# MMintLab/gelslim_depth

Measured on AMD Instinct MI355X. Metric: train frames/sec (320x427) at batch 32, higher is better.
Workload: dtype f32

## Files before the change

### gelslim_depth_amd/csrc/gsd_wgrad_w2d.hip

```cpp
#include "gsd_common.h"
#include "gsd_wgrad_internal.h"
#include <type_traits>

#include <cstdio>
#include <cstdlib>

typedef float f32x2d __attribute__((ext_vector_type(2)));

struct WgW2dParams {
  SrcD a0, a1;
  SrcD dy;
  float* slabs;
  int M, Ncols;
  int N, H, W;
  int KY, KX, kx_log2;
  int tiles_y, tiles_x, sy_n, sx_n;
  int WR, NP, NI;
  int ksteps_total, splits, mblocks, nblocks;
};

__device__ __forceinline__ float w2d_dpp(float v, const int ctrl_is_pair) {
  return ctrl_is_pair ? __builtin_bit_cast(float, __builtin_amdgcn_update_dpp(0, __builtin_bit_cast(int, v), 0xB1, 0xf, 0xf, true))
                      : __builtin_bit_cast(float, __builtin_amdgcn_update_dpp(0, __builtin_bit_cast(int, v), 0x5A, 0xf, 0xf, true));
}

template <int NWM, int NWN, bool PLAIN>
__global__ __launch_bounds__(512, 1) void wgrad3x3_w2d_kernel(const WgW2dParams P) {
  static_assert(NWM * NWN == 8, "8-wave blocks");
  constexpr int BM = 32 * NWM, BN = 16 * NWN;
  constexpr bool UROW = BM == 64;
  constexpr int NV = BN / 32;
  constexpr int TSU = BM * 24 + 4, TSV = BN * 24 + 4;
  constexpr int BUF = 4 * TSU + 4 * TSV;
  constexpr int NPD = UROW ? 1 : 2;
  constexpr int WINI = BN == 32 ? 10 : 20;
  constexpr int KB = BN == 32 ? 2 : 3;
  constexpr int WIN = NPD * 8 * 256;
  constexpr int IMG = WIN + 2 * WINI * 256;
  extern __shared__ __attribute__((aligned(16))) float smem[];

  const int tid = threadIdx.x, lane = tid & 63;
  const int wave = __builtin_amdgcn_readfirstlane(tid >> 6);
  const int wm = wave / NWN, wn = wave % NWN;
  const int j = lane >> 4, l16 = lane & 15;

  const int lid = xcd_swizzle(blockIdx.x, gridDim.x);
  const int per_split = P.mblocks * P.nblocks;
  const int split = lid / per_split;
  const int rem = lid - split * per_split;
  const int mb = rem % P.mblocks, nb = rem / P.mblocks;
  const int m0 = mb * BM, n0 = nb * BN;
  const int s_begin = (int)((long long)split * P.ksteps_total / P.splits);
  const int s_end = (int)((long long)(split + 1) * P.ksteps_total / P.splits);
  const int nst = s_end - s_begin;

  const bool seg1 = P.a1.C > 0 && n0 >= P.a0.C;
  const float* const S_p = seg1 ? P.a1.p : P.a0.p;
  const long long S_ns = seg1 ? P.a1.ns : P.a0.ns, S_cs = seg1 ? P.a1.cs : P.a0.cs;
  const int S_H = seg1 ? P.a1.H : P.a0.H, S_W = seg1 ? P.a1.W : P.a0.W, S_ws = seg1 ? P.a1.ws : P.a0.ws;
  const int S_oh = seg1 ? P.a1.oh : P.a0.oh, S_ow = seg1 ? P.a1.ow : P.a0.ow;
  const int S_c0 = n0 - (seg1 ? P.a0.C : 0);

  const int kxm = P.KX - 1;
  const int u_t = UROW ? (tid >> 1) & 3 : tid & 3;
  const int u_r = UROW ? tid & 1 : 0;
  const int u_co = UROW ? tid >> 3 : tid >> 2;
  const int u_tyl = u_t >> P.kx_log2, u_txl = u_t & kxm;
  const unsigned u_voff = (unsigned)((long long)u_co * P.dy.cs + (long long)(2 * u_tyl + u_r) * P.dy.ws + 4 * u_txl) * 4u;
  const unsigned u_wr = (unsigned)(IMG + u_t * TSU + u_co * 24) * 4u;
  const int v_kr = tid & 3, v_t = (tid >> 2) & 3, v_ci = tid >> 4;
  const int v_tyl = v_t >> P.kx_log2, v_txl = v_t & kxm;
  const unsigned v_rd = (unsigned)(WIN + ((v_ci * P.WR + 2 * v_tyl + v_kr) * P.NP + v_txl) * 4) * 4u;
  const unsigned v_wr = (unsigned)(IMG + 4 * TSU + v_t * TSV + v_ci * 24 + v_kr * 6) * 4u;
  int geo_packed = u_tyl | u_txl << 3 | v_tyl << 6 | v_txl << 9 | v_kr << 12 | u_r << 15;
  asm volatile("" : "+v"(geo_packed));
  const float v_sgn = (tid & 3) == 1 ? 1.f : -1.f;
  const float u_sgn = (UROW && (tid & 1)) ? -1.f : 1.f;
  constexpr int SCS = IMG + 2 * BUF;
  float lo = -__builtin_inff();
  if constexpr (!PLAIN) {
    const SrcD& S = seg1 ? P.a1 : P.a0;
    if (tid < BN) {
      f32x2d v = f32x2d{1.f, 0.f};
      if (S.scale != nullptr) v = f32x2d{S.scale[S_c0 + tid], S.shift[S_c0 + tid]};
      *reinterpret_cast<f32x2d*>(smem + SCS + 2 * tid) = v;
    }
    if (S.relu) lo = 0.f;
  }

  int st_n, st_sy, st_sx;
  {
    const int per = P.sy_n * P.sx_n;
    st_n = s_begin / per;
    const int rs = s_begin - st_n * per;
    st_sy = rs / P.sx_n;
    st_sx = rs - st_sy * P.sx_n;
  }

  int r_mask = 0;
  bool r_edge = false;
  float* const raw_w = smem + wave * 256;
  const float* const raw_r = smem + wave * 256 + lane * 4;
  unsigned x_off[KB];
  int x_meta = 0;
  {
    const int per_ch = P.WR * P.NP;
#pragma unroll
    for (int k = 0; k < KB; ++k) {
      const int pid = 64 * (wave + 8 * k) + lane;
      const int ch = pid / per_ch, rem = pid - ch * per_ch;
      const int wr = rem / P.NP, pp = rem - wr * P.NP;
      const bool dummy = ch >= BN;
      x_off[k] = dummy ? 0u : (unsigned)((long long)ch * S_cs + (long long)wr * S_ws + 4 * pp) * 4u;
      x_meta |= (dummy ? 128 : (wr | pp << 4)) << (8 * k);
    }
    asm volatile("" : "+v"(x_meta));
  }

  auto load = [&](auto wb_c) __attribute__((always_inline)) {
    constexpr int wb = decltype(wb_c)::value;
    const int n = st_n, ty0 = st_sy * P.KY, tx0 = st_sx * P.KX;
    if (++st_sx == P.sx_n) {
      st_sx = 0;
      if (++st_sy == P.sy_n) {
        st_sy = 0;
        ++st_n;
      }
    }
    const char* const dblk = reinterpret_cast<const char*>(P.dy.p + (long long)n * P.dy.ns + (long long)m0 * P.dy.cs);
    const char* vblk = reinterpret_cast<const char*>(S_p + (long long)n * S_ns + (long long)S_c0 * S_cs) - 16;
    asm volatile("" : "+s"(vblk));
    const int hs = 2 * ty0 - 1 - S_oh, wsx = 4 * tx0 - 1 - S_ow;
    const unsigned d_org = (unsigned)(2 * ty0 * P.dy.ws + 4 * tx0) * 4u;
    const int v_org = (hs * S_ws + wsx) * 4 + 16;
    const bool tiles_in = ty0 + P.KY <= P.tiles_y && tx0 + P.KX <= P.tiles_x;
    const bool inside = tiles_in && 2 * (ty0 + P.KY) <= P.H && hs >= 0 && hs + 2 * P.KY + 2 <= S_H && wsx >= 0 &&
                        wsx + 4 * P.KX + 2 <= S_W;
    r_edge = !inside;
    unsigned o_y0 = d_org + u_voff, o_y1 = o_y0 + (unsigned)P.dy.ws * 4u;
    if (!inside) {
      int m = 0;
      int geo = geo_packed;
      asm volatile("" : "+v"(geo));
      {
        const int ty = ty0 + (geo & 7), tx = tx0 + (geo >> 3 & 7);
        const bool t_ok = ty < P.tiles_y && tx < P.tiles_x;
        const int h = 2 * ty + (geo >> 15 & 1);
        const bool ok0 = t_ok && h < P.H, ok1 = t_ok && h + 1 < P.H;
        o_y0 = ok0 ? o_y0 : 0u;
        o_y1 = ok1 ? o_y1 : 0u;
        m = (ok0 ? 1 : 0) | (ok1 ? 2 : 0);
      }
      {
        const int vy = geo >> 6 & 7, vx = geo >> 9 & 7;
        const int ty = ty0 + vy, tx = tx0 + vx;
        const bool t_ok = ty < P.tiles_y && tx < P.tiles_x;
        const int row = hs + 2 * vy + (geo >> 12 & 3), c0 = wsx + 4 * vx;
        const bool r_ok = t_ok && (unsigned)row < (unsigned)S_H;
        const int lo_ = c0 < 0 ? -c0 : 0, hi_ = S_W - c0;
        const int lo = lo_ < 6 ? lo_ : 6, hi = hi_ < 0 ? 0 : (hi_ < 6 ? hi_ : 6);
        const int cm = (r_ok && hi > lo) ? ((1 << hi) - 1) & ~((1 << lo) - 1) : 0;
        m |= cm << 2;
      }
      r_mask = m;
    }
    auto fill = [&](const char* base, unsigned off, float* dst) __attribute__((always_inline)) {
      __builtin_amdgcn_global_load_lds(reinterpret_cast<const float*>(base + off), dst, 16, 0, 0);
    };
#pragma unroll
    for (int k = 0; k < KB; ++k)
      if (wave + 8 * k < P.NI) {
        unsigned off = (unsigned)v_org + x_off[k];
        if (!inside) {
          int mt = x_meta;
          asm volatile("" : "+v"(mt));
          mt >>= 8 * k;
          const int row = hs + (mt & 15), c0 = wsx + 4 * (mt >> 4 & 7);
          const bool ok = !(mt & 128) && (unsigned)row < (unsigned)S_H && c0 + 3 >= 0 && c0 < S_W;
          off = ok ? off : 0u;
        }
        fill(vblk, off, smem + WIN + wb * (WINI * 256) + (wave + 8 * k) * 256);
      }
    __builtin_amdgcn_s_waitcnt(0xC07F);
    fill(dblk, o_y0, raw_w);
    if constexpr (!UROW) fill(dblk, o_y1, raw_w + 8 * 256);
  };

  auto transform = [&](auto buf_c) __attribute__((always_inline)) {
    constexpr int buf = decltype(buf_c)::value;
    const f32x2d p1m1 = {1.f, -1.f}, p2m2 = {2.f, -2.f}, c4 = {4.f, 4.f};
    auto a4_row = [&](const f32x4& y, f32x2d& u12, f32x2d& u34) __attribute__((always_inline)) {
      const f32x2d lo2 = {y[0], y[1]}, hi2 = {y[2], y[3]};
      const f32x2d pq = lo2 + hi2;
      const f32x2d ab = __builtin_elementwise_fma(c4, hi2, lo2);
      u12 = __builtin_elementwise_fma(f32x2d{pq[1], pq[1]}, p1m1, f32x2d{pq[0], pq[0]});
      u34 = __builtin_elementwise_fma(f32x2d{ab[1], ab[1]}, p2m2, f32x2d{ab[0], ab[0]});
    };
    {
      f32x4 y0 = *reinterpret_cast<const f32x4*>(raw_r), y1 = y0;
      if constexpr (!UROW) y1 = *reinterpret_cast<const f32x4*>(raw_r + 8 * 256);
      if (r_edge) {
        if (!(r_mask & 1)) y0 = f32x4{0.f, 0.f, 0.f, 0.f};
        if constexpr (!UROW)
          if (!(r_mask & 2)) y1 = f32x4{0.f, 0.f, 0.f, 0.f};
      }
      f32x2d a12, a34;
      a4_row(y0, a12, a34);
      if constexpr (UROW) {
        const f32x2d sg = {u_sgn, u_sgn};
        const f32x2d a05 = {y0[0], y0[3]};
        const f32x2d x12 = {w2d_dpp(a12[0], 1), w2d_dpp(a12[1], 1)}, x34 = {w2d_dpp(a34[0], 1), w2d_dpp(a34[1], 1)};
        const f32x2d x05 = {w2d_dpp(a05[0], 1), w2d_dpp(a05[1], 1)};
        const f32x2d t12 = __builtin_elementwise_fma(a12, sg, x12), t34 = __builtin_elementwise_fma(a34, sg, x34);
        const f32x2d t05 = __builtin_elementwise_fma(a05, sg, x05);
        float* const o_own = reinterpret_cast<float*>(reinterpret_cast<char*>(smem) + u_wr) + buf * BUF + ((tid & 1) ? 18 : 0);
        float* const o_t1 = reinterpret_cast<float*>(reinterpret_cast<char*>(smem) + u_wr) + buf * BUF + ((tid & 1) ? 12 : 6);
        *reinterpret_cast<f32x2d*>(o_own) = a12;
        *reinterpret_cast<f32x2d*>(o_own + 2) = a34;
        *reinterpret_cast<f32x2d*>(o_own + 4) = a05;
        *reinterpret_cast<f32x2d*>(o_t1) = t12;
        *reinterpret_cast<f32x2d*>(o_t1 + 2) = t34;
        *reinterpret_cast<f32x2d*>(o_t1 + 4) = t05;
      } else {
        f32x2d b12, b34;
        a4_row(y1, b12, b34);
        const f32x2d s12 = a12 + b12, s34 = a34 + b34, d12 = a12 - b12, d34 = a34 - b34;
        const float s0 = y0[0] + y1[0], s5 = y0[3] + y1[3], d0 = y0[0] - y1[0], d5 = y0[3] - y1[3];
        float* const op = reinterpret_cast<float*>(reinterpret_cast<char*>(smem) + u_wr) + buf * BUF;
        *reinterpret_cast<f32x4*>(op) = f32x4{a12[0], a12[1], a34[0], a34[1]};
        *reinterpret_cast<f32x4*>(op + 4) = f32x4{y0[0], y0[3], s12[0], s12[1]};
        *reinterpret_cast<f32x4*>(op + 8) = f32x4{s34[0], s34[1], s0, s5};
        *reinterpret_cast<f32x4*>(op + 12) = f32x4{d12[0], d12[1], d34[0], d34[1]};
        *reinterpret_cast<f32x4*>(op + 16) = f32x4{d0, d5, b12[0], b12[1]};
        *reinterpret_cast<f32x4*>(op + 20) = f32x4{b34[0], b34[1], y1[0], y1[3]};
      }
    }
#pragma unroll
    for (int i = 0; i < NV; ++i) {
      const float* const wp = reinterpret_cast<const float*>(reinterpret_cast<const char*>(smem) + v_rd) + buf * (WINI * 256) + i * 32 * (P.WR * P.NP * 4);
      const f32x4 ra = *reinterpret_cast<const f32x4*>(wp);
      const f32x2d rb = *reinterpret_cast<const f32x2d*>(wp + 4);
      f32x2d t0 = {ra[0], ra[1]}, t1 = {ra[2], ra[3]}, t2 = rb;
      if constexpr (!PLAIN) {
        const f32x2d ss = *reinterpret_cast<const f32x2d*>(smem + SCS + 2 * ((tid >> 4) + 32 * i));
        const f32x2d sc2 = {ss[0], ss[0]}, sh2 = {ss[1], ss[1]}, lo2 = {lo, lo};
        t0 = __builtin_elementwise_max(__builtin_elementwise_fma(t0, sc2, sh2), lo2);
        t1 = __builtin_elementwise_max(__builtin_elementwise_fma(t1, sc2, sh2), lo2);
        t2 = __builtin_elementwise_max(__builtin_elementwise_fma(t2, sc2, sh2), lo2);
      }
      if (r_edge) {
        const int m = r_mask;
        if (!(m & 4)) t0[0] = 0.f;
        if (!(m & 8)) t0[1] = 0.f;
        if (!(m & 16)) t1[0] = 0.f;
        if (!(m & 32)) t1[1] = 0.f;
        if (!(m & 64)) t2[0] = 0.f;
        if (!(m & 128)) t2[1] = 0.f;
      }
      const f32x2d m41 = {-4.f, -1.f}, m5 = {-5.f, -5.f};
      const f32x2d ac = __builtin_elementwise_fma(f32x2d{t1[0], t1[0]}, m41, f32x2d{t2[0], t2[0]});
      const f32x2d be = __builtin_elementwise_fma(f32x2d{t0[1], t0[1]}, m41, f32x2d{t1[1], t1[1]});
      const f32x2d v12 = __builtin_elementwise_fma(f32x2d{be[0], be[0]}, p1m1, f32x2d{ac[0], ac[0]});
      const f32x2d v34 = __builtin_elementwise_fma(f32x2d{be[1], be[1]}, p2m2, f32x2d{ac[1], ac[1]});
      const f32x2d v05 = __builtin_elementwise_fma(t0, c4, __builtin_elementwise_fma(t1, m5, t2));
      const f32x2d sg = {v_sgn, v_sgn};
      const f32x2d x12 = {w2d_dpp(v12[0], 0), w2d_dpp(v12[1], 0)}, x34 = {w2d_dpp(v34[0], 0), w2d_dpp(v34[1], 0)};
      const f32x2d x05 = {w2d_dpp(v05[0], 0), w2d_dpp(v05[1], 0)};
      float* const op = reinterpret_cast<float*>(reinterpret_cast<char*>(smem) + v_wr) + buf * BUF + i * (32 * 24);
      *reinterpret_cast<f32x2d*>(op) = __builtin_elementwise_fma(sg, x12, v12);
      *reinterpret_cast<f32x2d*>(op + 2) = __builtin_elementwise_fma(sg, x34, v34);
      *reinterpret_cast<f32x2d*>(op + 4) = __builtin_elementwise_fma(sg, x05, v05);
    }
  };

  f32x4 acc[2][24];

  const int a_rd = IMG + j * TSU + (wm * 32 + l16) * 24;
  const int b_rd = IMG + 4 * TSU + j * TSV + (wn * 16 + l16) * 24;

  using I0 = std::integral_constant<int, 0>;
  using I1 = std::integral_constant<int, 1>;
  if (nst > 0) {
    load(I0{});
    gsd_dma_barrier();
    transform(I0{});
    if (nst > 1) load(I1{});
    gsd_dma_barrier();
  }
#pragma unroll
  for (int m = 0; m < 2; ++m)
#pragma unroll
    for (int f = 0; f < 24; ++f) acc[m][f] = f32x4{0.f, 0.f, 0.f, 0.f};
  if (nst > 0) {
    auto step = [&](const int it, auto cur_c) __attribute__((always_inline)) {
      constexpr int cur = decltype(cur_c)::value, nxt = cur ^ 1;
      const bool tr = it + 1 < nst, ld = it + 2 < nst;
      const float* const Sb = smem + cur * BUF;
      const f32x2d p1m1 = {1.f, -1.f}, p2m2 = {2.f, -2.f}, c4 = {4.f, 4.f};
      f32x4 a0, a1, b;
      auto rd_ops = [&](const int g) __attribute__((always_inline)) {
        a0 = *reinterpret_cast<const f32x4*>(Sb + a_rd + 4 * g);
        a1 = *reinterpret_cast<const f32x4*>(Sb + a_rd + 16 * 24 + 4 * g);
        b = *reinterpret_cast<const f32x4*>(Sb + b_rd + 4 * g);
      };
      auto mm = [&](const int g) __attribute__((always_inline)) {
#pragma unroll
        for (int e = 0; e < 4; ++e) {
          acc[0][4 * g + e] = mfma16(a0[e], b[e], acc[0][4 * g + e]);
          acc[1][4 * g + e] = mfma16(a1[e], b[e], acc[1][4 * g + e]);
        }
      };
      auto a4_row = [&](const f32x4& y, f32x2d& u12, f32x2d& u34) __attribute__((always_inline)) {
        const f32x2d lo2 = {y[0], y[1]}, hi2 = {y[2], y[3]};
        const f32x2d pq = lo2 + hi2;
        const f32x2d ab = __builtin_elementwise_fma(c4, hi2, lo2);
        u12 = __builtin_elementwise_fma(f32x2d{pq[1], pq[1]}, p1m1, f32x2d{pq[0], pq[0]});
        u34 = __builtin_elementwise_fma(f32x2d{ab[1], ab[1]}, p2m2, f32x2d{ab[0], ab[0]});
      };
      const int t_mask = r_mask;
      const bool t_edge = r_edge;
      f32x4 y0, y1;
      f32x2d a12, a34, b12, b34;
      f32x4 ra;
      f32x2d rb, v12, v34, v05;
      float* const u_out = reinterpret_cast<float*>(reinterpret_cast<char*>(smem) + u_wr) + nxt * BUF;
      auto rd_y = [&]() __attribute__((always_inline)) {
        y0 = *reinterpret_cast<const f32x4*>(raw_r);
        y1 = y0;
        if constexpr (!UROW) y1 = *reinterpret_cast<const f32x4*>(raw_r + 8 * 256);
      };
      auto u_rows = [&]() __attribute__((always_inline)) {
        if (t_edge) {
          if (!(t_mask & 1)) y0 = f32x4{0.f, 0.f, 0.f, 0.f};
          if constexpr (!UROW)
            if (!(t_mask & 2)) y1 = f32x4{0.f, 0.f, 0.f, 0.f};
        }
        a4_row(y0, a12, a34);
        if constexpr (!UROW) a4_row(y1, b12, b34);
      };
      auto u_cols = [&]() __attribute__((always_inline)) {
        if constexpr (UROW) {
          const f32x2d sg = {u_sgn, u_sgn};
          const f32x2d a05 = {y0[0], y0[3]};
          const f32x2d x12 = {w2d_dpp(a12[0], 1), w2d_dpp(a12[1], 1)}, x34 = {w2d_dpp(a34[0], 1), w2d_dpp(a34[1], 1)};
          const f32x2d x05 = {w2d_dpp(a05[0], 1), w2d_dpp(a05[1], 1)};
          float* const o_own = u_out + ((tid & 1) ? 18 : 0);
          float* const o_t1 = u_out + ((tid & 1) ? 12 : 6);
          *reinterpret_cast<f32x2d*>(o_own) = a12;
          *reinterpret_cast<f32x2d*>(o_own + 2) = a34;
          *reinterpret_cast<f32x2d*>(o_own + 4) = a05;
          *reinterpret_cast<f32x2d*>(o_t1) = __builtin_elementwise_fma(a12, sg, x12);
          *reinterpret_cast<f32x2d*>(o_t1 + 2) = __builtin_elementwise_fma(a34, sg, x34);
          *reinterpret_cast<f32x2d*>(o_t1 + 4) = __builtin_elementwise_fma(a05, sg, x05);
        } else {
          const f32x2d s12 = a12 + b12, s34 = a34 + b34, d12 = a12 - b12, d34 = a34 - b34;
          const float s0 = y0[0] + y1[0], s5 = y0[3] + y1[3], d0 = y0[0] - y1[0], d5 = y0[3] - y1[3];
          *reinterpret_cast<f32x4*>(u_out) = f32x4{a12[0], a12[1], a34[0], a34[1]};
          *reinterpret_cast<f32x4*>(u_out + 4) = f32x4{y0[0], y0[3], s12[0], s12[1]};
          *reinterpret_cast<f32x4*>(u_out + 8) = f32x4{s34[0], s34[1], s0, s5};
          *reinterpret_cast<f32x4*>(u_out + 12) = f32x4{d12[0], d12[1], d34[0], d34[1]};
          *reinterpret_cast<f32x4*>(u_out + 16) = f32x4{d0, d5, b12[0], b12[1]};
          *reinterpret_cast<f32x4*>(u_out + 20) = f32x4{b34[0], b34[1], y1[0], y1[3]};
        }
      };
      auto rd_v = [&](const int i) __attribute__((always_inline)) {
        const float* const wp = reinterpret_cast<const float*>(reinterpret_cast<const char*>(smem) + v_rd) + nxt * (WINI * 256) + i * 32 * (P.WR * P.NP * 4);
        ra = *reinterpret_cast<const f32x4*>(wp);
        rb = *reinterpret_cast<const f32x2d*>(wp + 4);
      };
      auto v_rows = [&](const int i) __attribute__((always_inline)) {
        f32x2d t0 = {ra[0], ra[1]}, t1 = {ra[2], ra[3]}, t2 = rb;
        if constexpr (!PLAIN) {
          const f32x2d ss = *reinterpret_cast<const f32x2d*>(smem + SCS + 2 * ((tid >> 4) + 32 * i));
          const f32x2d sc2 = {ss[0], ss[0]}, sh2 = {ss[1], ss[1]}, lo2 = {lo, lo};
          t0 = __builtin_elementwise_max(__builtin_elementwise_fma(t0, sc2, sh2), lo2);
          t1 = __builtin_elementwise_max(__builtin_elementwise_fma(t1, sc2, sh2), lo2);
          t2 = __builtin_elementwise_max(__builtin_elementwise_fma(t2, sc2, sh2), lo2);
        }
        if (t_edge) {
          const int m = t_mask;
          if (!(m & 4)) t0[0] = 0.f;
          if (!(m & 8)) t0[1] = 0.f;
          if (!(m & 16)) t1[0] = 0.f;
          if (!(m & 32)) t1[1] = 0.f;
          if (!(m & 64)) t2[0] = 0.f;
          if (!(m & 128)) t2[1] = 0.f;
        }
        const f32x2d m41 = {-4.f, -1.f}, m5 = {-5.f, -5.f};
        const f32x2d ac = __builtin_elementwise_fma(f32x2d{t1[0], t1[0]}, m41, f32x2d{t2[0], t2[0]});
        const f32x2d be = __builtin_elementwise_fma(f32x2d{t0[1], t0[1]}, m41, f32x2d{t1[1], t1[1]});
        v12 = __builtin_elementwise_fma(f32x2d{be[0], be[0]}, p1m1, f32x2d{ac[0], ac[0]});
        v34 = __builtin_elementwise_fma(f32x2d{be[1], be[1]}, p2m2, f32x2d{ac[1], ac[1]});
        v05 = __builtin_elementwise_fma(t0, c4, __builtin_elementwise_fma(t1, m5, t2));
      };
      auto v_cols = [&](const int i) __attribute__((always_inline)) {
        int tq = threadIdx.x;
        asm volatile("" : "+v"(tq));
        const float sgn = (tq & 3) == 1 ? 1.f : -1.f;
        const f32x2d sg = {sgn, sgn};
        const f32x2d x12 = {w2d_dpp(v12[0], 0), w2d_dpp(v12[1], 0)}, x34 = {w2d_dpp(v34[0], 0), w2d_dpp(v34[1], 0)};
        const f32x2d x05 = {w2d_dpp(v05[0], 0), w2d_dpp(v05[1], 0)};
        float* const op = reinterpret_cast<float*>(reinterpret_cast<char*>(smem) + v_wr) + nxt * BUF + i * (32 * 24);
        *reinterpret_cast<f32x2d*>(op) = __builtin_elementwise_fma(sg, x12, v12);
        *reinterpret_cast<f32x2d*>(op + 2) = __builtin_elementwise_fma(sg, x34, v34);
        *reinterpret_cast<f32x2d*>(op + 4) = __builtin_elementwise_fma(sg, x05, v05);
      };
      auto group = [&](const int g, auto piece) __attribute__((always_inline)) {
        mm(g);
        __builtin_amdgcn_sched_barrier(0);
        if (g + 1 < 6) rd_ops(g + 1);
        piece();
        __builtin_amdgcn_sched_barrier(0);
      };
      rd_ops(0);
      if (tr) rd_y();
      __builtin_amdgcn_sched_barrier(0);
      group(0, [&]() __attribute__((always_inline)) { if (ld) load(cur_c); });
      group(1, [&]() __attribute__((always_inline)) { if (tr) { u_rows(); if constexpr (UROW) u_cols(); } });
      group(2, [&]() __attribute__((always_inline)) { if (tr) { rd_v(0); if constexpr (!UROW) u_cols(); } });
      group(3, [&]() __attribute__((always_inline)) { if (tr) v_rows(0); });
      group(4, [&]() __attribute__((always_inline)) { if (tr) { v_cols(0); if constexpr (NV > 1) rd_v(1); } });
      group(5, [&]() __attribute__((always_inline)) {
        if constexpr (NV > 1) {
          if (tr) { v_rows(1); v_cols(1); }
        }
      });
      gsd_dma_barrier();
    };
    for (int it = 0; it < nst; it += 2) {
      step(it, I0{});
      if (it + 1 < nst) step(it + 1, I1{});
    }
  }

  const size_t pl = (size_t)P.M * P.Ncols;
  int tid_e = threadIdx.x;
  asm volatile("" : "+v"(tid_e));
  const int j_e = (tid_e & 63) >> 4, l16_e = tid_e & 15;
#pragma unroll
  for (int m = 0; m < 2; ++m)
#pragma unroll
    for (int reg = 0; reg < 4; ++reg) {
      const int mr = m0 + wm * 32 + m * 16 + j_e * 4 + reg;
      const int col = n0 + wn * 16 + l16_e;
      float E[4][3];
#pragma unroll
      for (int fr = 0; fr < 4; ++fr) {
        const float D1 = acc[m][fr * 6 + 0][reg], D2 = acc[m][fr * 6 + 1][reg], D3 = acc[m][fr * 6 + 2][reg];
        const float D4 = acc[m][fr * 6 + 3][reg], D0 = acc[m][fr * 6 + 4][reg], D5 = acc[m][fr * 6 + 5][reg];
        E[fr][0] = 0.25f * D0 - (1.f / 6.f) * (D1 + D2) + (1.f / 24.f) * (D3 + D4);
        E[fr][1] = (1.f / 6.f) * (D2 - D1) + (1.f / 12.f) * (D3 - D4);
        E[fr][2] = (1.f / 6.f) * (D3 + D4 - D1 - D2) + D5;
      }
      float* const o = P.slabs + ((size_t)split * 9 * P.M + mr) * P.Ncols + col;
#pragma unroll
      for (int s = 0; s < 3; ++s) {
        const float h = 0.5f * (E[1][s] + E[2][s]);
        o[(0 * 3 + s) * pl] = E[0][s] + h;
        o[(1 * 3 + s) * pl] = 0.5f * (E[1][s] - E[2][s]);
        o[(2 * 3 + s) * pl] = h + E[3][s];
      }
    }
}

namespace {

struct WgW2dPlan {
  int KY, KX, kx_log2, tiles_y, tiles_x, sy_n, sx_n, BM, BN, mblocks, nblocks, ksteps_total, splits;
  int64_t slab_elems;
  bool ok;
};

WgW2dPlan plan_wg2d(int N, int H, int W, int M, int Ncols) {
  WgW2dPlan p;
  p.tiles_y = ceil_div(H, 2);
  p.tiles_x = ceil_div(W, 4);
  long best = -1;
  const int force_kx = gsd_env_int("GSD_WG2D_KX", 0);
  for (int kx = 4; kx >= 1; kx /= 2) {
    if (force_kx && kx != force_kx) continue;
    const int ky = 4 / kx;
    const long steps = (long)ceil_div(p.tiles_y, ky) * ceil_div(p.tiles_x, kx) * (kx == 4 ? 100 : kx == 2 ? 99 : 112);
    if (best < 0 || steps < best) {
      best = steps;
      p.KY = ky; p.KX = kx;
    }
  }
  p.kx_log2 = p.KX == 4 ? 2 : p.KX == 2 ? 1 : 0;
  p.sy_n = ceil_div(p.tiles_y, p.KY);
  p.sx_n = ceil_div(p.tiles_x, p.KX);
  p.BM = M >= 128 ? 128 : 64;
  p.BN = p.BM == 128 ? 32 : 64;
  p.ok = M % p.BM == 0 && Ncols % p.BN == 0;
  p.mblocks = ceil_div(M, p.BM);
  p.nblocks = ceil_div(Ncols, p.BN);
  p.ksteps_total = N * p.sy_n * p.sx_n;
  const int target = gsd_env_int("GSD_WG2D_BLOCKS", 256);
  int splits = ceil_div(target, p.mblocks * p.nblocks);
  if (splits > p.ksteps_total) splits = p.ksteps_total;
  if (splits > 2048) splits = 2048;
  if (splits < 1) splits = 1;
  p.splits = splits;
  p.slab_elems = (int64_t)splits * 9 * M * Ncols;
  return p;
}

}

int64_t gsd_wgrad_w2d_workspace(int N, int H, int W, int Cin, int Cout) {
  const WgW2dPlan p = plan_wg2d(N, H, W, Cout, Cin);
  return p.ok ? p.slab_elems : 0;
}

int64_t gsd_wgrad_w2d_mfma_count(int N, int H, int W, int Cin, int Cout) {
  const WgW2dPlan p = plan_wg2d(N, H, W, Cout, Cin);
  return p.ok ? (int64_t)p.ksteps_total * 24 * (Cout / 16) * (Cin / 16) : 0;
}

int gsd_wgrad_w2d_use(const gsd_src* a, int nsrc, const gsd_src* dy, int Cin, int Cout, int N, int H, int W) {
  if (gsd_env_int("GSD_WGRAD_W2D", 1) == 0) return 0;
  const WgW2dPlan p = plan_wg2d(N, H, W, Cout, Cin);
  if (!p.ok) return 0;
  if (dy->w_stride % 4 != 0 || ((uintptr_t)dy->ptr & 15) != 0 || dy->c_stride % 4 != 0 || dy->n_stride % 4 != 0) return 0;
  if (dy->w_stride < 4 * p.tiles_x) return 0;
  if ((int64_t)p.BM * dy->c_stride * 4 >= (1LL << 31)) return 0;
  if (nsrc == 2 && a[0].C % p.BN != 0) return 0;
  for (int i = 0; i < nsrc; ++i) {
    if (a[i].slack < 4) return 0;
    if ((int64_t)p.BN * a[i].c_stride * 4 >= (1LL << 31)) return 0;
    if ((int64_t)(a[i].H + 4) * a[i].w_stride * 4 >= (1LL << 31)) return 0;
  }
  return 1;
}

int gsd_wgrad_w2d_run(const gsd_src* a, int nsrc, const gsd_src* dy, int Cin, int Cout, float* workspace, int64_t workspace_elems,
                      int N, int H, int W, int* splits_out, void* stream) {
  const WgW2dPlan pl = plan_wg2d(N, H, W, Cout, Cin);
  GSD_REQUIRE(pl.ok, GSD_ERR_UNSUPPORTED, "gsd_conv3x3_wgrad (w2d): shape not served");
  GSD_REQUIRE(workspace_elems >= pl.slab_elems, GSD_ERR_WORKSPACE, "gsd_conv3x3_wgrad: workspace %lld < %lld elements",
              (long long)workspace_elems, (long long)pl.slab_elems);
  WgW2dParams P;
  P.a0 = to_srcd(a[0]);
  P.a1 = nsrc > 1 ? to_srcd(a[1]) : null_srcd();
  P.dy = to_srcd(*dy);
  P.slabs = workspace;
  P.M = Cout; P.Ncols = Cin;
  P.N = N; P.H = H; P.W = W;
  P.KY = pl.KY; P.KX = pl.KX; P.kx_log2 = pl.kx_log2;
  P.tiles_y = pl.tiles_y; P.tiles_x = pl.tiles_x; P.sy_n = pl.sy_n; P.sx_n = pl.sx_n;
  P.WR = 2 * pl.KY + 2; P.NP = pl.KX + 1;
  P.NI = (pl.BN * P.WR * P.NP + 63) / 64;
  P.ksteps_total = pl.ksteps_total; P.splits = pl.splits; P.mblocks = pl.mblocks; P.nblocks = pl.nblocks;
  bool plain = true;
  for (int i = 0; i < nsrc; ++i) plain = plain && a[i].scale == nullptr && a[i].relu == 0;
  const long grid = (long)pl.splits * pl.mblocks * pl.nblocks;
  const size_t lds = ((size_t)(pl.BM == 64 ? 1 : 2) * 8 * 256 + (size_t)2 * (pl.BN == 32 ? 10 : 20) * 256 +
                      (size_t)2 * (4 * (pl.BM * 24 + 4) + 4 * (pl.BN * 24 + 4)) + 2 * pl.BN) * sizeof(float);
  GSD_REQUIRE(P.NI <= 8 * (pl.BN == 32 ? 2 : 3) && P.NI <= (pl.BN == 32 ? 10 : 20), GSD_ERR_UNSUPPORTED, "gsd_conv3x3_wgrad (w2d): window image too large");
  if (gsd_env_set("GSD_WG43_TRACE"))
    fprintf(stderr, "wg2d M%d N%d %dx%d B%d kstep %dx%d ksteps %d splits %d blocks %ld BM %d BN %d plain %d lds %zu\n", Cout, Cin, H, W,
            N, pl.KY, pl.KX, pl.ksteps_total, pl.splits, grid, pl.BM, pl.BN, (int)plain, lds);
  const dim3 g((int)grid);
  const hipStream_t st = (hipStream_t)stream;
  const char* const what = "gsd_conv3x3_wgrad (w2d)";
  if (int e = pl.BM == 128 ? (plain ? gsd_launch<wgrad3x3_w2d_kernel<4, 2, true>>(what, g, dim3(512), lds, st, P)
                                    : gsd_launch<wgrad3x3_w2d_kernel<4, 2, false>>(what, g, dim3(512), lds, st, P))
                           : (plain ? gsd_launch<wgrad3x3_w2d_kernel<2, 4, true>>(what, g, dim3(512), lds, st, P)
                                    : gsd_launch<wgrad3x3_w2d_kernel<2, 4, false>>(what, g, dim3(512), lds, st, P)))
    return e;
  *splits_out = pl.splits;
  return GSD_OK;
}
```

Measured before the change: 382.5.

## Precompute edge masks, branchless load masking, and restructure LDS transform stores in Winograd wgrad

Replaces per-step boundary checks in the Winograd 3x3 weight-gradient kernel with per-thread row/column mask tables computed once. Each k-step is classified as first, last or second-to-last, and zeroing is done with bitwise masks instead of branches. The U/V transform stores are reorganised into a new LDS record layout addressed through raw LDS pointers, and the epilogue is remapped to match. The step loop drops its per-iteration tr/ld guards, and the default block target becomes the CU count. The code adds stricter eligibility checks on source offsets and NI, and carries a correctness risk if the remapped layout or mask tables miss a boundary case.

```diff
diff --git a/gelslim_depth_amd/csrc/gsd_wgrad_w2d.hip b/gelslim_depth_amd/csrc/gsd_wgrad_w2d.hip
--- a/gelslim_depth_amd/csrc/gsd_wgrad_w2d.hip
+++ b/gelslim_depth_amd/csrc/gsd_wgrad_w2d.hip
@@ -6,6 +6,11 @@
 #include <cstdlib>
 
 typedef float f32x2d __attribute__((ext_vector_type(2)));
+
+template <class T>
+__device__ __forceinline__ __attribute__((address_space(3))) T* wg_lds(unsigned byte_addr) {
+  return (__attribute__((address_space(3))) T*)(size_t)byte_addr;
+}
 
 struct WgW2dParams {
   SrcD a0, a1;
@@ -18,6 +23,20 @@
   int WR, NP, NI;
   int ksteps_total, splits, mblocks, nblocks;
 };
+
+__device__ __forceinline__ int wg_bit_mask(int m, const int bit) {
+  int k = (m << (31 - bit)) >> 31;
+  asm volatile("" : "+v"(k));
+  return k;
+}
+__device__ __forceinline__ float wg_keep(float x, int m, const int bit) {
+  return __builtin_bit_cast(float, __builtin_bit_cast(int, x) & wg_bit_mask(m, bit));
+}
+__device__ __forceinline__ f32x4 wg_keep4(const f32x4 x, int m, const int bit) {
+  typedef int i32x4w __attribute__((ext_vector_type(4)));
+  const int k = wg_bit_mask(m, bit);
+  return __builtin_bit_cast(f32x4, __builtin_bit_cast(i32x4w, x) & i32x4w{k, k, k, k});
+}
 
 __device__ __forceinline__ float w2d_dpp(float v, const int ctrl_is_pair) {
   return ctrl_is_pair ? __builtin_bit_cast(float, __builtin_amdgcn_update_dpp(0, __builtin_bit_cast(int, v), 0xB1, 0xf, 0xf, true))
@@ -66,16 +85,20 @@
   const int u_r = UROW ? tid & 1 : 0;
   const int u_co = UROW ? tid >> 3 : tid >> 2;
   const int u_tyl = u_t >> P.kx_log2, u_txl = u_t & kxm;
-  const unsigned u_voff = (unsigned)((long long)u_co * P.dy.cs + (long long)(2 * u_tyl + u_r) * P.dy.ws + 4 * u_txl) * 4u;
-  const unsigned u_wr = (unsigned)(IMG + u_t * TSU + u_co * 24) * 4u;
+  unsigned u_voff = (unsigned)((long long)u_co * P.dy.cs + (long long)(2 * u_tyl + u_r) * P.dy.ws + 4 * u_txl) * 4u;
+  const unsigned smem_b = (unsigned)(size_t)(__attribute__((address_space(3))) void*)smem;
+  const unsigned u_rec = smem_b + (unsigned)(IMG + u_t * TSU + u_co * 24) * 4u;
+  const unsigned u_wr = u_rec + (UROW ? 16u * u_r : 0u);
+  const unsigned u_ws = u_rec + 64u + 4u * u_r;
   const int v_kr = tid & 3, v_t = (tid >> 2) & 3, v_ci = tid >> 4;
   const int v_tyl = v_t >> P.kx_log2, v_txl = v_t & kxm;
-  const unsigned v_rd = (unsigned)(WIN + ((v_ci * P.WR + 2 * v_tyl + v_kr) * P.NP + v_txl) * 4) * 4u;
-  const unsigned v_wr = (unsigned)(IMG + 4 * TSU + v_t * TSV + v_ci * 24 + v_kr * 6) * 4u;
-  int geo_packed = u_tyl | u_txl << 3 | v_tyl << 6 | v_txl << 9 | v_kr << 12 | u_r << 15;
-  asm volatile("" : "+v"(geo_packed));
-  const float v_sgn = (tid & 3) == 1 ? 1.f : -1.f;
-  const float u_sgn = (UROW && (tid & 1)) ? -1.f : 1.f;
+  const unsigned v_rd = smem_b + (unsigned)(WIN + ((v_ci * P.WR + 2 * v_tyl + v_kr) * P.NP + v_txl) * 4) * 4u;
+  const int v_slot = (0x1320 >> (4 * v_kr)) & 3;
+  const unsigned v_rec = smem_b + (unsigned)(IMG + 4 * TSU + v_t * TSV + v_ci * 24) * 4u;
+  const unsigned v_wr = v_rec + 16u * v_slot;
+  const unsigned v_ws = v_rec + 64u + 16u * (v_slot >> 1) + 4u * (v_slot & 1);
+  float v_sgn = (tid & 3) == 1 ? 1.f : -1.f;
+  float u_sgn = (UROW && (tid & 1)) ? -1.f : 1.f;
   constexpr int SCS = IMG + 2 * BUF;
   float lo = -__builtin_inff();
   if constexpr (!PLAIN) {
@@ -98,12 +121,17 @@
   }
 
   int r_mask = 0;
-  bool r_edge = false;
+  int r_edge = 0;
+  int st_left = nst - 1;
   float* const raw_w = smem + wave * 256;
   const float* const raw_r = smem + wave * 256 + lane * 4;
   unsigned x_off[KB];
-  int x_meta = 0;
+  auto fill_bit = [](const int k) { return k < 2 ? 256 << k : 2; };
+  int row_tab, col_tab;
+  const int sy_l2 = P.sy_n > 2 && 2 * (P.sy_n - 1) * P.KY + 1 - S_oh > S_H ? P.sy_n - 2 : -1;
+  const int sx_l2 = P.sx_n > 2 && 4 * (P.sx_n - 1) * P.KX + 1 - S_ow > S_W ? P.sx_n - 2 : -1;
   {
+    int x_wr[KB], x_pp[KB];
     const int per_ch = P.WR * P.NP;
 #pragma unroll
     for (int k = 0; k < KB; ++k) {
@@ -112,20 +140,57 @@
       const int wr = rem / P.NP, pp = rem - wr * P.NP;
       const bool dummy = ch >= BN;
       x_off[k] = dummy ? 0u : (unsigned)((long long)ch * S_cs + (long long)wr * S_ws + 4 * pp) * 4u;
-      x_meta |= (dummy ? 128 : (wr | pp << 4)) << (8 * k);
-    }
-    asm volatile("" : "+v"(x_meta));
+      x_wr[k] = dummy ? -1 : wr;
+      x_pp[k] = pp;
+    }
+    auto row_field = [&](const int ty0) {
+      const int hs = 2 * ty0 - 1 - S_oh;
+      const int uty = ty0 + u_tyl, h = 2 * uty + u_r;
+      int f = (uty < P.tiles_y && h < P.H ? 1 : 0) | (!UROW && uty < P.tiles_y && h + 1 < P.H ? 2 : 0);
+      if (ty0 + v_tyl < P.tiles_y && (unsigned)(hs + 2 * v_tyl + v_kr) < (unsigned)S_H) f |= 0xFC;
+#pragma unroll
+      for (int k = 0; k < KB; ++k)
+        if (x_wr[k] >= 0 && (unsigned)(hs + x_wr[k]) < (unsigned)S_H) f |= fill_bit(k);
+      return f;
+    };
+    auto col_field = [&](const int tx0) {
+      const int wsx = 4 * tx0 - 1 - S_ow;
+      int f = tx0 + u_txl < P.tiles_x ? (UROW ? 1 : 3) : 0;
+      const int c0 = wsx + 4 * v_txl;
+      const int lo_ = c0 < 0 ? -c0 : 0, hi_ = S_W - c0;
+      const int lo = lo_ < 6 ? lo_ : 6, hi = hi_ < 0 ? 0 : (hi_ < 6 ? hi_ : 6);
+      if (tx0 + v_txl < P.tiles_x && hi > lo) f |= (((1 << hi) - 1) & ~((1 << lo) - 1)) << 2;
+#pragma unroll
+      for (int k = 0; k < KB; ++k) {
+        const int ck = wsx + 4 * x_pp[k];
+        if (x_wr[k] >= 0 && ck + 3 >= 0 && ck < S_W) f |= fill_bit(k);
+      }
+      return f;
+    };
+    row_tab = row_field(0) | row_field((P.sy_n - 1) * P.KY) << 10 | row_field((P.sy_n > 2 ? P.sy_n - 2 : 0) * P.KY) << 20;
+    col_tab = col_field(0) | col_field((P.sx_n - 1) * P.KX) << 10 | col_field((P.sx_n > 2 ? P.sx_n - 2 : 0) * P.KX) << 20;
+    asm volatile("" : "+v"(row_tab), "+v"(col_tab));
   }
 
+  auto fill_on = [&](const int k) __attribute__((always_inline)) {
+    if (k < KB - 1) return true;
+    int w = wave;
+    asm volatile("" : "+s"(w));
+    return w + 8 * (KB - 1) < P.NI;
+  };
   auto load = [&](auto wb_c) __attribute__((always_inline)) {
     constexpr int wb = decltype(wb_c)::value;
     const int n = st_n, ty0 = st_sy * P.KY, tx0 = st_sx * P.KX;
-    if (++st_sx == P.sx_n) {
-      st_sx = 0;
-      if (++st_sy == P.sy_n) {
-        st_sy = 0;
-        ++st_n;
-      }
+    const int cy = st_sy == 0 ? 1 : (st_sy == P.sy_n - 1 ? 2 : (st_sy == sy_l2 ? 3 : 0));
+    const int cx = st_sx == 0 ? 1 : (st_sx == P.sx_n - 1 ? 2 : (st_sx == sx_l2 ? 3 : 0));
+    {
+      const int adv = st_left > 0 ? 1 : 0;
+      st_left -= adv;
+      const int sx1 = st_sx + 1, wx = sx1 == P.sx_n ? 1 : 0;
+      const int sy1 = st_sy + wx, wy = sy1 == P.sy_n ? 1 : 0;
+      st_sx = adv ? (wx ? 0 : sx1) : st_sx;
+      st_sy = adv ? (wy ? 0 : sy1) : st_sy;
+      st_n += adv & wy;
     }
     const char* const dblk = reinterpret_cast<const char*>(P.dy.p + (long long)n * P.dy.ns + (long long)m0 * P.dy.cs);
     const char* vblk = reinterpret_cast<const char*>(S_p + (long long)n * S_ns + (long long)S_c0 * S_cs) - 16;
@@ -133,35 +198,18 @@
     const int hs = 2 * ty0 - 1 - S_oh, wsx = 4 * tx0 - 1 - S_ow;
     const unsigned d_org = (unsigned)(2 * ty0 * P.dy.ws + 4 * tx0) * 4u;
     const int v_org = (hs * S_ws + wsx) * 4 + 16;
-    const bool tiles_in = ty0 + P.KY <= P.tiles_y && tx0 + P.KX <= P.tiles_x;
-    const bool inside = tiles_in && 2 * (ty0 + P.KY) <= P.H && hs >= 0 && hs + 2 * P.KY + 2 <= S_H && wsx >= 0 &&
-                        wsx + 4 * P.KX + 2 <= S_W;
-    r_edge = !inside;
-    unsigned o_y0 = d_org + u_voff, o_y1 = o_y0 + (unsigned)P.dy.ws * 4u;
-    if (!inside) {
-      int m = 0;
-      int geo = geo_packed;
-      asm volatile("" : "+v"(geo));
-      {
-        const int ty = ty0 + (geo & 7), tx = tx0 + (geo >> 3 & 7);
-        const bool t_ok = ty < P.tiles_y && tx < P.tiles_x;
-        const int h = 2 * ty + (geo >> 15 & 1);
-        const bool ok0 = t_ok && h < P.H, ok1 = t_ok && h + 1 < P.H;
-        o_y0 = ok0 ? o_y0 : 0u;
-        o_y1 = ok1 ? o_y1 : 0u;
-        m = (ok0 ? 1 : 0) | (ok1 ? 2 : 0);
-      }
-      {
-        const int vy = geo >> 6 & 7, vx = geo >> 9 & 7;
-        const int ty = ty0 + vy, tx = tx0 + vx;
-        const bool t_ok = ty < P.tiles_y && tx < P.tiles_x;
-        const int row = hs + 2 * vy + (geo >> 12 & 3), c0 = wsx + 4 * vx;
-        const bool r_ok = t_ok && (unsigned)row < (unsigned)S_H;
-        const int lo_ = c0 < 0 ? -c0 : 0, hi_ = S_W - c0;
-        const int lo = lo_ < 6 ? lo_ : 6, hi = hi_ < 0 ? 0 : (hi_ < 6 ? hi_ : 6);
-        const int cm = (r_ok && hi > lo) ? ((1 << hi) - 1) & ~((1 << lo) - 1) : 0;
-        m |= cm << 2;
-      }
+    r_edge = __builtin_amdgcn_readfirstlane(cy | cx);
+    asm volatile("" : "+v"(u_voff));
+    unsigned o_y0 = d_org + u_voff, o_y1 = d_org + (unsigned)P.dy.ws * 4u + u_voff;
+    unsigned x_o[KB];
+#pragma unroll
+    for (int k = 0; k < KB; ++k) x_o[k] = (unsigned)v_org + x_off[k];
+    if (__builtin_expect(r_edge != 0, 0)) {
+      const int m = ((row_tab >> (cy ? 10 * cy - 10 : 0)) | (cy ? 0 : 0x3ff)) & ((col_tab >> (cx ? 10 * cx - 10 : 0)) | (cx ? 0 : 0x3ff));
+      o_y0 &= (unsigned)wg_bit_mask(m, 0);
+      if constexpr (!UROW) o_y1 &= (unsigned)wg_bit_mask(m, 1);
+#pragma unroll
+      for (int k = 0; k < KB; ++k) x_o[k] &= (unsigned)wg_bit_mask(m, k < 2 ? 8 + k : 1);
       r_mask = m;
     }
     auto fill = [&](const char* base, unsigned off, float* dst) __attribute__((always_inline)) {
@@ -169,21 +217,51 @@
     };
 #pragma unroll
     for (int k = 0; k < KB; ++k)
-      if (wave + 8 * k < P.NI) {
-        unsigned off = (unsigned)v_org + x_off[k];
-        if (!inside) {
-          int mt = x_meta;
-          asm volatile("" : "+v"(mt));
-          mt >>= 8 * k;
-          const int row = hs + (mt & 15), c0 = wsx + 4 * (mt >> 4 & 7);
-          const bool ok = !(mt & 128) && (unsigned)row < (unsigned)S_H && c0 + 3 >= 0 && c0 < S_W;
-          off = ok ? off : 0u;
-        }
-        fill(vblk, off, smem + WIN + wb * (WINI * 256) + (wave + 8 * k) * 256);
+      if (fill_on(k)) {
+        fill(vblk, x_o[k], smem + WIN + wb * (WINI * 256) + (wave + 8 * k) * 256);
       }
     __builtin_amdgcn_s_waitcnt(0xC07F);
     fill(dblk, o_y0, raw_w);
     if constexpr (!UROW) fill(dblk, o_y1, raw_w + 8 * 256);
+  };
+
+  auto st1 = [&](const unsigned a, const float v) __attribute__((always_inline)) { *wg_lds<volatile float>(a) = v; };
+  auto st_u = [&](const unsigned ib, const f32x4& y0, const f32x4& y1, const f32x2d a12, const f32x2d a34, const f32x2d b12,
+                  const f32x2d b34) __attribute__((always_inline)) {
+    if constexpr (UROW) {
+      asm volatile("" : "+v"(u_sgn));
+      const float sgn = u_sgn;
+      const f32x2d sg = {sgn, sgn};
+      const f32x2d x12 = {w2d_dpp(a12[0], 1), w2d_dpp(a12[1], 1)}, x34 = {w2d_dpp(a34[0], 1), w2d_dpp(a34[1], 1)};
+      const float x0 = w2d_dpp(y0[0], 1), x5 = w2d_dpp(y0[3], 1);
+      const f32x2d t12 = __builtin_elementwise_fma(a12, sg, x12), t34 = __builtin_elementwise_fma(a34, sg, x34);
+      *wg_lds<f32x4>(u_wr + ib) = f32x4{a12[0], a12[1], a34[0], a34[1]};
+      *wg_lds<f32x4>(u_wr + ib + 32) = f32x4{t12[0], t12[1], t34[0], t34[1]};
+      st1(u_ws + ib, y0[0]);
+      st1(u_ws + ib + 8, y0[3]);
+      st1(u_ws + ib + 16, __builtin_fmaf(y0[0], sgn, x0));
+      st1(u_ws + ib + 24, __builtin_fmaf(y0[3], sgn, x5));
+    } else {
+      const f32x2d pm = {1.f, -1.f};
+      const f32x2d sd0 = __builtin_elementwise_fma(f32x2d{y1[0], y1[0]}, pm, f32x2d{y0[0], y0[0]});
+      const f32x2d sd5 = __builtin_elementwise_fma(f32x2d{y1[3], y1[3]}, pm, f32x2d{y0[3], y0[3]});
+      *wg_lds<f32x2d>(u_wr + ib) = a12;
+      *wg_lds<f32x2d>(u_wr + ib + 8) = a34;
+      *wg_lds<f32x2d>(u_wr + ib + 16) = b12;
+      *wg_lds<f32x2d>(u_wr + ib + 24) = b34;
+      *wg_lds<f32x2d>(u_wr + ib + 32) = a12 + b12;
+      *wg_lds<f32x2d>(u_wr + ib + 40) = a34 + b34;
+      *wg_lds<f32x2d>(u_wr + ib + 48) = a12 - b12;
+      *wg_lds<f32x2d>(u_wr + ib + 56) = a34 - b34;
+      *wg_lds<f32x4>(u_wr + ib + 64) = f32x4{y0[0], y1[0], y0[3], y1[3]};
+      *wg_lds<f32x2d>(u_wr + ib + 80) = sd0;
+      *wg_lds<f32x2d>(u_wr + ib + 88) = sd5;
+    }
+  };
+  auto st_v = [&](const unsigned ib, const f32x2d o12, const f32x2d o34, const f32x2d o05) __attribute__((always_inline)) {
+    *wg_lds<f32x4>(v_wr + ib) = f32x4{o12[0], o12[1], o34[0], o34[1]};
+    st1(v_ws + ib, o05[0]);
+    st1(v_ws + ib + 8, o05[1]);
   };
 
   auto transform = [&](auto buf_c) __attribute__((always_inline)) {
@@ -200,46 +278,20 @@
       f32x4 y0 = *reinterpret_cast<const f32x4*>(raw_r), y1 = y0;
       if constexpr (!UROW) y1 = *reinterpret_cast<const f32x4*>(raw_r + 8 * 256);
       if (r_edge) {
-        if (!(r_mask & 1)) y0 = f32x4{0.f, 0.f, 0.f, 0.f};
-        if constexpr (!UROW)
-          if (!(r_mask & 2)) y1 = f32x4{0.f, 0.f, 0.f, 0.f};
+        y0 = wg_keep4(y0, r_mask, 0);
+        if constexpr (!UROW) y1 = wg_keep4(y1, r_mask, 1);
       }
       f32x2d a12, a34;
       a4_row(y0, a12, a34);
-      if constexpr (UROW) {
-        const f32x2d sg = {u_sgn, u_sgn};
-        const f32x2d a05 = {y0[0], y0[3]};
-        const f32x2d x12 = {w2d_dpp(a12[0], 1), w2d_dpp(a12[1], 1)}, x34 = {w2d_dpp(a34[0], 1), w2d_dpp(a34[1], 1)};
-        const f32x2d x05 = {w2d_dpp(a05[0], 1), w2d_dpp(a05[1], 1)};
-        const f32x2d t12 = __builtin_elementwise_fma(a12, sg, x12), t34 = __builtin_elementwise_fma(a34, sg, x34);
-        const f32x2d t05 = __builtin_elementwise_fma(a05, sg, x05);
-        float* const o_own = reinterpret_cast<float*>(reinterpret_cast<char*>(smem) + u_wr) + buf * BUF + ((tid & 1) ? 18 : 0);
-        float* const o_t1 = reinterpret_cast<float*>(reinterpret_cast<char*>(smem) + u_wr) + buf * BUF + ((tid & 1) ? 12 : 6);
-        *reinterpret_cast<f32x2d*>(o_own) = a12;
-        *reinterpret_cast<f32x2d*>(o_own + 2) = a34;
-        *reinterpret_cast<f32x2d*>(o_own + 4) = a05;
-        *reinterpret_cast<f32x2d*>(o_t1) = t12;
-        *reinterpret_cast<f32x2d*>(o_t1 + 2) = t34;
-        *reinterpret_cast<f32x2d*>(o_t1 + 4) = t05;
-      } else {
-        f32x2d b12, b34;
-        a4_row(y1, b12, b34);
-        const f32x2d s12 = a12 + b12, s34 = a34 + b34, d12 = a12 - b12, d34 = a34 - b34;
-        const float s0 = y0[0] + y1[0], s5 = y0[3] + y1[3], d0 = y0[0] - y1[0], d5 = y0[3] - y1[3];
-        float* const op = reinterpret_cast<float*>(reinterpret_cast<char*>(smem) + u_wr) + buf * BUF;
-        *reinterpret_cast<f32x4*>(op) = f32x4{a12[0], a12[1], a34[0], a34[1]};
-        *reinterpret_cast<f32x4*>(op + 4) = f32x4{y0[0], y0[3], s12[0], s12[1]};
-        *reinterpret_cast<f32x4*>(op + 8) = f32x4{s34[0], s34[1], s0, s5};
-        *reinterpret_cast<f32x4*>(op + 12) = f32x4{d12[0], d12[1], d34[0], d34[1]};
-        *reinterpret_cast<f32x4*>(op + 16) = f32x4{d0, d5, b12[0], b12[1]};
-        *reinterpret_cast<f32x4*>(op + 20) = f32x4{b34[0], b34[1], y1[0], y1[3]};
-      }
+      f32x2d b12 = a12, b34 = a34;
+      if constexpr (!UROW) a4_row(y1, b12, b34);
+      st_u(buf * BUF * 4u, y0, y1, a12, a34, b12, b34);
     }
 #pragma unroll
     for (int i = 0; i < NV; ++i) {
-      const float* const wp = reinterpret_cast<const float*>(reinterpret_cast<const char*>(smem) + v_rd) + buf * (WINI * 256) + i * 32 * (P.WR * P.NP * 4);
-      const f32x4 ra = *reinterpret_cast<const f32x4*>(wp);
-      const f32x2d rb = *reinterpret_cast<const f32x2d*>(wp + 4);
+      const unsigned wp = v_rd + buf * (WINI * 256) * 4u + (i ? (unsigned)(32 * 16 * (P.WR * P.NP)) : 0u);
+      const f32x4 ra = *wg_lds<const f32x4>(wp);
+      const f32x2d rb = *wg_lds<const f32x2d>(wp + 16);
       f32x2d t0 = {ra[0], ra[1]}, t1 = {ra[2], ra[3]}, t2 = rb;
       if constexpr (!PLAIN) {
         const f32x2d ss = *reinterpret_cast<const f32x2d*>(smem + SCS + 2 * ((tid >> 4) + 32 * i));
@@ -250,12 +302,9 @@
       }
       if (r_edge) {
         const int m = r_mask;
-        if (!(m & 4)) t0[0] = 0.f;
-        if (!(m & 8)) t0[1] = 0.f;
-        if (!(m & 16)) t1[0] = 0.f;
-        if (!(m & 32)) t1[1] = 0.f;
-        if (!(m & 64)) t2[0] = 0.f;
-        if (!(m & 128)) t2[1] = 0.f;
+        t0 = f32x2d{wg_keep(t0[0], m, 2), wg_keep(t0[1], m, 3)};
+        t1 = f32x2d{wg_keep(t1[0], m, 4), wg_keep(t1[1], m, 5)};
+        t2 = f32x2d{wg_keep(t2[0], m, 6), wg_keep(t2[1], m, 7)};
       }
       const f32x2d m41 = {-4.f, -1.f}, m5 = {-5.f, -5.f};
       const f32x2d ac = __builtin_elementwise_fma(f32x2d{t1[0], t1[0]}, m41, f32x2d{t2[0], t2[0]});
@@ -266,17 +315,17 @@
       const f32x2d sg = {v_sgn, v_sgn};
       const f32x2d x12 = {w2d_dpp(v12[0], 0), w2d_dpp(v12[1], 0)}, x34 = {w2d_dpp(v34[0], 0), w2d_dpp(v34[1], 0)};
       const f32x2d x05 = {w2d_dpp(v05[0], 0), w2d_dpp(v05[1], 0)};
-      float* const op = reinterpret_cast<float*>(reinterpret_cast<char*>(smem) + v_wr) + buf * BUF + i * (32 * 24);
-      *reinterpret_cast<f32x2d*>(op) = __builtin_elementwise_fma(sg, x12, v12);
-      *reinterpret_cast<f32x2d*>(op + 2) = __builtin_elementwise_fma(sg, x34, v34);
-      *reinterpret_cast<f32x2d*>(op + 4) = __builtin_elementwise_fma(sg, x05, v05);
+      st_v((buf * BUF + i * (32 * 24)) * 4u, __builtin_elementwise_fma(sg, x12, v12), __builtin_elementwise_fma(sg, x34, v34),
+           __builtin_elementwise_fma(sg, x05, v05));
     }
   };
 
   f32x4 acc[2][24];
 
-  const int a_rd = IMG + j * TSU + (wm * 32 + l16) * 24;
-  const int b_rd = IMG + 4 * TSU + j * TSV + (wn * 16 + l16) * 24;
+  unsigned a_rd = smem_b + (unsigned)(IMG + j * TSU + (wm * 32 + l16) * 24) * 4u;
+  unsigned b_rd = smem_b + (unsigned)(IMG + 4 * TSU + j * TSV + (wn * 16 + l16) * 24) * 4u;
+  asm volatile("" : "+v"(a_rd), "+v"(b_rd));
+  static_assert((BUF + 16 * 24 + 24) * 4 < 65536, "image 1 within the 16-bit offset of a ds_read");
 
   using I0 = std::integral_constant<int, 0>;
   using I1 = std::integral_constant<int, 1>;
@@ -284,7 +333,7 @@
     load(I0{});
     gsd_dma_barrier();
     transform(I0{});
-    if (nst > 1) load(I1{});
+    load(I1{});
     gsd_dma_barrier();
   }
 #pragma unroll
@@ -292,16 +341,14 @@
 #pragma unroll
     for (int f = 0; f < 24; ++f) acc[m][f] = f32x4{0.f, 0.f, 0.f, 0.f};
   if (nst > 0) {
-    auto step = [&](const int it, auto cur_c) __attribute__((always_inline)) {
+    auto step = [&](auto cur_c) __attribute__((always_inline)) {
       constexpr int cur = decltype(cur_c)::value, nxt = cur ^ 1;
-      const bool tr = it + 1 < nst, ld = it + 2 < nst;
-      const float* const Sb = smem + cur * BUF;
       const f32x2d p1m1 = {1.f, -1.f}, p2m2 = {2.f, -2.f}, c4 = {4.f, 4.f};
       f32x4 a0, a1, b;
       auto rd_ops = [&](const int g) __attribute__((always_inline)) {
-        a0 = *reinterpret_cast<const f32x4*>(Sb + a_rd + 4 * g);
-        a1 = *reinterpret_cast<const f32x4*>(Sb + a_rd + 16 * 24 + 4 * g);
-        b = *reinterpret_cast<const f32x4*>(Sb + b_rd + 4 * g);
+        a0 = *wg_lds<const f32x4>(a_rd + (cur * BUF + 4 * g) * 4u);
+        a1 = *wg_lds<const f32x4>(a_rd + (cur * BUF + 16 * 24 + 4 * g) * 4u);
+        b = *wg_lds<const f32x4>(b_rd + (cur * BUF + 4 * g) * 4u);
       };
       auto mm = [&](const int g) __attribute__((always_inline)) {
 #pragma unroll
@@ -318,55 +365,37 @@
         u34 = __builtin_elementwise_fma(f32x2d{ab[1], ab[1]}, p2m2, f32x2d{ab[0], ab[0]});
       };
       const int t_mask = r_mask;
-      const bool t_edge = r_edge;
+      int t_edge = r_edge;
+      asm volatile("" : "+s"(t_edge));
+      auto edge = [&]() __attribute__((always_inline)) {
+        int e = t_edge;
+        asm volatile("" : "+s"(e));
+        return e != 0;
+      };
       f32x4 y0, y1;
       f32x2d a12, a34, b12, b34;
       f32x4 ra;
       f32x2d rb, v12, v34, v05;
-      float* const u_out = reinterpret_cast<float*>(reinterpret_cast<char*>(smem) + u_wr) + nxt * BUF;
       auto rd_y = [&]() __attribute__((always_inline)) {
         y0 = *reinterpret_cast<const f32x4*>(raw_r);
         y1 = y0;
         if constexpr (!UROW) y1 = *reinterpret_cast<const f32x4*>(raw_r + 8 * 256);
       };
       auto u_rows = [&]() __attribute__((always_inline)) {
-        if (t_edge) {
-          if (!(t_mask & 1)) y0 = f32x4{0.f, 0.f, 0.f, 0.f};
-          if constexpr (!UROW)
-            if (!(t_mask & 2)) y1 = f32x4{0.f, 0.f, 0.f, 0.f};
+        if (__builtin_expect(edge(), 0)) {
+          y0 = wg_keep4(y0, t_mask, 0);
+          if constexpr (!UROW) y1 = wg_keep4(y1, t_mask, 1);
         }
         a4_row(y0, a12, a34);
         if constexpr (!UROW) a4_row(y1, b12, b34);
       };
       auto u_cols = [&]() __attribute__((always_inline)) {
-        if constexpr (UROW) {
-          const f32x2d sg = {u_sgn, u_sgn};
-          const f32x2d a05 = {y0[0], y0[3]};
-          const f32x2d x12 = {w2d_dpp(a12[0], 1), w2d_dpp(a12[1], 1)}, x34 = {w2d_dpp(a34[0], 1), w2d_dpp(a34[1], 1)};
-          const f32x2d x05 = {w2d_dpp(a05[0], 1), w2d_dpp(a05[1], 1)};
-          float* const o_own = u_out + ((tid & 1) ? 18 : 0);
-          float* const o_t1 = u_out + ((tid & 1) ? 12 : 6);
-          *reinterpret_cast<f32x2d*>(o_own) = a12;
-          *reinterpret_cast<f32x2d*>(o_own + 2) = a34;
-          *reinterpret_cast<f32x2d*>(o_own + 4) = a05;
-          *reinterpret_cast<f32x2d*>(o_t1) = __builtin_elementwise_fma(a12, sg, x12);
-          *reinterpret_cast<f32x2d*>(o_t1 + 2) = __builtin_elementwise_fma(a34, sg, x34);
-          *reinterpret_cast<f32x2d*>(o_t1 + 4) = __builtin_elementwise_fma(a05, sg, x05);
-        } else {
-          const f32x2d s12 = a12 + b12, s34 = a34 + b34, d12 = a12 - b12, d34 = a34 - b34;
-          const float s0 = y0[0] + y1[0], s5 = y0[3] + y1[3], d0 = y0[0] - y1[0], d5 = y0[3] - y1[3];
-          *reinterpret_cast<f32x4*>(u_out) = f32x4{a12[0], a12[1], a34[0], a34[1]};
-          *reinterpret_cast<f32x4*>(u_out + 4) = f32x4{y0[0], y0[3], s12[0], s12[1]};
-          *reinterpret_cast<f32x4*>(u_out + 8) = f32x4{s34[0], s34[1], s0, s5};
-          *reinterpret_cast<f32x4*>(u_out + 12) = f32x4{d12[0], d12[1], d34[0], d34[1]};
-          *reinterpret_cast<f32x4*>(u_out + 16) = f32x4{d0, d5, b12[0], b12[1]};
-          *reinterpret_cast<f32x4*>(u_out + 20) = f32x4{b34[0], b34[1], y1[0], y1[3]};
-        }
+        st_u(nxt * BUF * 4u, y0, y1, a12, a34, b12, b34);
       };
       auto rd_v = [&](const int i) __attribute__((always_inline)) {
-        const float* const wp = reinterpret_cast<const float*>(reinterpret_cast<const char*>(smem) + v_rd) + nxt * (WINI * 256) + i * 32 * (P.WR * P.NP * 4);
-        ra = *reinterpret_cast<const f32x4*>(wp);
-        rb = *reinterpret_cast<const f32x2d*>(wp + 4);
+        const unsigned wp = v_rd + nxt * (WINI * 256) * 4u + (i ? (unsigned)(32 * 16 * (P.WR * P.NP)) : 0u);
+        ra = *wg_lds<const f32x4>(wp);
+        rb = *wg_lds<const f32x2d>(wp + 16);
       };
       auto v_rows = [&](const int i) __attribute__((always_inline)) {
         f32x2d t0 = {ra[0], ra[1]}, t1 = {ra[2], ra[3]}, t2 = rb;
@@ -377,14 +406,11 @@
           t1 = __builtin_elementwise_max(__builtin_elementwise_fma(t1, sc2, sh2), lo2);
           t2 = __builtin_elementwise_max(__builtin_elementwise_fma(t2, sc2, sh2), lo2);
         }
-        if (t_edge) {
+        if (__builtin_expect(edge(), 0)) {
           const int m = t_mask;
-          if (!(m & 4)) t0[0] = 0.f;
-          if (!(m & 8)) t0[1] = 0.f;
-          if (!(m & 16)) t1[0] = 0.f;
-          if (!(m & 32)) t1[1] = 0.f;
-          if (!(m & 64)) t2[0] = 0.f;
-          if (!(m & 128)) t2[1] = 0.f;
+          t0 = f32x2d{wg_keep(t0[0], m, 2), wg_keep(t0[1], m, 3)};
+          t1 = f32x2d{wg_keep(t1[0], m, 4), wg_keep(t1[1], m, 5)};
+          t2 = f32x2d{wg_keep(t2[0], m, 6), wg_keep(t2[1], m, 7)};
         }
         const f32x2d m41 = {-4.f, -1.f}, m5 = {-5.f, -5.f};
         const f32x2d ac = __builtin_elementwise_fma(f32x2d{t1[0], t1[0]}, m41, f32x2d{t2[0], t2[0]});
@@ -394,16 +420,12 @@
         v05 = __builtin_elementwise_fma(t0, c4, __builtin_elementwise_fma(t1, m5, t2));
       };
       auto v_cols = [&](const int i) __attribute__((always_inline)) {
-        int tq = threadIdx.x;
-        asm volatile("" : "+v"(tq));
-        const float sgn = (tq & 3) == 1 ? 1.f : -1.f;
-        const f32x2d sg = {sgn, sgn};
+        asm volatile("" : "+v"(v_sgn));
+        const f32x2d sg = {v_sgn, v_sgn};
         const f32x2d x12 = {w2d_dpp(v12[0], 0), w2d_dpp(v12[1], 0)}, x34 = {w2d_dpp(v34[0], 0), w2d_dpp(v34[1], 0)};
         const f32x2d x05 = {w2d_dpp(v05[0], 0), w2d_dpp(v05[1], 0)};
-        float* const op = reinterpret_cast<float*>(reinterpret_cast<char*>(smem) + v_wr) + nxt * BUF + i * (32 * 24);
-        *reinterpret_cast<f32x2d*>(op) = __builtin_elementwise_fma(sg, x12, v12);
-        *reinterpret_cast<f32x2d*>(op + 2) = __builtin_elementwise_fma(sg, x34, v34);
-        *reinterpret_cast<f32x2d*>(op + 4) = __builtin_elementwise_fma(sg, x05, v05);
+        st_v((nxt * BUF + i * (32 * 24)) * 4u, __builtin_elementwise_fma(sg, x12, v12), __builtin_elementwise_fma(sg, x34, v34),
+             __builtin_elementwise_fma(sg, x05, v05));
       };
       auto group = [&](const int g, auto piece) __attribute__((always_inline)) {
         mm(g);
@@ -413,23 +435,24 @@
         __builtin_amdgcn_sched_barrier(0);
       };
       rd_ops(0);
-      if (tr) rd_y();
+      rd_y();
       __builtin_amdgcn_sched_barrier(0);
-      group(0, [&]() __attribute__((always_inline)) { if (ld) load(cur_c); });
-      group(1, [&]() __attribute__((always_inline)) { if (tr) { u_rows(); if constexpr (UROW) u_cols(); } });
-      group(2, [&]() __attribute__((always_inline)) { if (tr) { rd_v(0); if constexpr (!UROW) u_cols(); } });
-      group(3, [&]() __attribute__((always_inline)) { if (tr) v_rows(0); });
-      group(4, [&]() __attribute__((always_inline)) { if (tr) { v_cols(0); if constexpr (NV > 1) rd_v(1); } });
+      group(0, [&]() __attribute__((always_inline)) { load(cur_c); });
+      group(1, [&]() __attribute__((always_inline)) { u_rows(); if constexpr (UROW) u_cols(); });
+      group(2, [&]() __attribute__((always_inline)) { rd_v(0); if constexpr (!UROW) u_cols(); });
+      group(3, [&]() __attribute__((always_inline)) { v_rows(0); });
+      group(4, [&]() __attribute__((always_inline)) { v_cols(0); if constexpr (NV > 1) rd_v(1); });
       group(5, [&]() __attribute__((always_inline)) {
         if constexpr (NV > 1) {
-          if (tr) { v_rows(1); v_cols(1); }
+          v_rows(1);
+          v_cols(1);
         }
       });
       gsd_dma_barrier();
     };
     for (int it = 0; it < nst; it += 2) {
-      step(it, I0{});
-      if (it + 1 < nst) step(it + 1, I1{});
+      step(I0{});
+      if (it + 1 < nst) step(I1{});
     }
   }
 
@@ -446,8 +469,9 @@
       float E[4][3];
 #pragma unroll
       for (int fr = 0; fr < 4; ++fr) {
-        const float D1 = acc[m][fr * 6 + 0][reg], D2 = acc[m][fr * 6 + 1][reg], D3 = acc[m][fr * 6 + 2][reg];
-        const float D4 = acc[m][fr * 6 + 3][reg], D0 = acc[m][fr * 6 + 4][reg], D5 = acc[m][fr * 6 + 5][reg];
+        const int sl = (0x1320 >> (4 * fr)) & 3, f0 = 16 + 4 * (sl >> 1) + (sl & 1);
+        const float D1 = acc[m][4 * sl + 0][reg], D2 = acc[m][4 * sl + 1][reg], D3 = acc[m][4 * sl + 2][reg];
+        const float D4 = acc[m][4 * sl + 3][reg], D0 = acc[m][f0][reg], D5 = acc[m][f0 + 2][reg];
         E[fr][0] = 0.25f * D0 - (1.f / 6.f) * (D1 + D2) + (1.f / 24.f) * (D3 + D4);
         E[fr][1] = (1.f / 6.f) * (D2 - D1) + (1.f / 12.f) * (D3 - D4);
         E[fr][2] = (1.f / 6.f) * (D3 + D4 - D1 - D2) + D5;
@@ -476,7 +500,9 @@
   p.tiles_y = ceil_div(H, 2);
   p.tiles_x = ceil_div(W, 4);
   long best = -1;
-  const int force_kx = gsd_env_int("GSD_WG2D_KX", 0);
+  int force_kx = gsd_env_int("GSD_WG2D_KX", 0);
+  if (force_kx != 1 && force_kx != 2 && force_kx != 4) force_kx = 0;
+  p.KY = 1; p.KX = 4;
   for (int kx = 4; kx >= 1; kx /= 2) {
     if (force_kx && kx != force_kx) continue;
     const int ky = 4 / kx;
@@ -495,7 +521,7 @@
   p.mblocks = ceil_div(M, p.BM);
   p.nblocks = ceil_div(Ncols, p.BN);
   p.ksteps_total = N * p.sy_n * p.sx_n;
-  const int target = gsd_env_int("GSD_WG2D_BLOCKS", 256);
+  const int target = gsd_env_int("GSD_WG2D_BLOCKS", gsd_cu_count());
   int splits = ceil_div(target, p.mblocks * p.nblocks);
   if (splits > p.ksteps_total) splits = p.ksteps_total;
   if (splits > 2048) splits = 2048;
@@ -526,6 +552,8 @@
   if ((int64_t)p.BM * dy->c_stride * 4 >= (1LL << 31)) return 0;
   if (nsrc == 2 && a[0].C % p.BN != 0) return 0;
   for (int i = 0; i < nsrc; ++i) {
+    if (p.sy_n > 2 && (a[i].off_h < 0 || a[i].off_h > 2 * p.KY - 1 || 2 * (p.sy_n > 3 ? p.sy_n - 2 : 0) * p.KY + 1 - a[i].off_h > a[i].H)) return 0;
+    if (p.sx_n > 2 && (a[i].off_w < 0 || a[i].off_w > 4 * p.KX - 1 || 4 * (p.sx_n > 3 ? p.sx_n - 2 : 0) * p.KX + 1 - a[i].off_w > a[i].W)) return 0;
     if (a[i].slack < 4) return 0;
     if ((int64_t)p.BN * a[i].c_stride * 4 >= (1LL << 31)) return 0;
     if ((int64_t)(a[i].H + 4) * a[i].w_stride * 4 >= (1LL << 31)) return 0;
@@ -556,7 +584,7 @@
   const long grid = (long)pl.splits * pl.mblocks * pl.nblocks;
   const size_t lds = ((size_t)(pl.BM == 64 ? 1 : 2) * 8 * 256 + (size_t)2 * (pl.BN == 32 ? 10 : 20) * 256 +
                       (size_t)2 * (4 * (pl.BM * 24 + 4) + 4 * (pl.BN * 24 + 4)) + 2 * pl.BN) * sizeof(float);
-  GSD_REQUIRE(P.NI <= 8 * (pl.BN == 32 ? 2 : 3) && P.NI <= (pl.BN == 32 ? 10 : 20), GSD_ERR_UNSUPPORTED, "gsd_conv3x3_wgrad (w2d): window image too large");
+  GSD_REQUIRE(P.NI <= 8 * (pl.BN == 32 ? 2 : 3) && P.NI <= (pl.BN == 32 ? 10 : 20) && P.NI > 8 * (pl.BN == 32 ? 1 : 2), GSD_ERR_UNSUPPORTED, "gsd_conv3x3_wgrad (w2d): window image too large");
   if (gsd_env_set("GSD_WG43_TRACE"))
     fprintf(stderr, "wg2d M%d N%d %dx%d B%d kstep %dx%d ksteps %d splits %d blocks %ld BM %d BN %d plain %d lds %zu\n", Cout, Cin, H, W,
             N, pl.KY, pl.KX, pl.ksteps_total, pl.splits, grid, pl.BM, pl.BN, (int)plain, lds);
```

Result: faster. 389.6 (median of 6 runs) (+1.8%).
